# jmschrei/blueberry

Hardware: AMD Instinct MI355X
Metric: Gpair-updates/s per stress iteration, N=50k (higher is better)
Workload: dtype f32

## Files before the change

blueberry_amd/csrc/bb_solver.hip:

```cpp
#include <math.h>
#include <stddef.h>
#include <stdlib.h>
#include <string.h>
#include <time.h>
#include <unistd.h>

#include <algorithm>
#include <cmath>
#include <type_traits>
#include <vector>

#include <condition_variable>
#include <map>
#include <mutex>
#include <thread>
#include <tuple>

#include "bb_comm.h"
#include "bb_common.h"
#include "bb_group_barrier.h"
#include "bb_solver_kernels.h"

struct bb_solver {
    int dtype = BB_F32, device = 0, rank = 0, world = 1;
    bool wide = true;
    bb_layout_info L{};
    std::vector<int32_t> tile_I, tile_J;
    int64_t u_begin = 0, u_end = 0, n_local = 0;
    int64_t t_first = 0, n_local_tiles = 0;
    std::vector<int2> udesc;

    hipStream_t stream = nullptr;
    bool own_stream = false;
    bool stream_stuck = false;

    void *d_units = nullptr, *d_X = nullptr, *d_V = nullptr, *d_part = nullptr, *d_exch = nullptr;
    double momentum = 0.0;
    bool own_exch = false;
    int2 *d_udesc = nullptr;
    int chunk_q = 0, chunk_r = 0;
    bool nontemporal = true;
    char *d_arena = nullptr;
    int2 *d_wave_slots = nullptr;
    int lds_wave_floats = 0;
    double *d_stresspart = nullptr;
    double *d_stress_slot = nullptr;
    std::vector<int32_t> slot_strip;
    std::vector<int32_t> wave_last_strip;
    int n_maps = 1;
    void *d_bin_scale = nullptr;
    int *d_map_ptr = nullptr, *d_map_idx = nullptr;
    double *d_map_scalar = nullptr;
    std::vector<int64_t> map_begin;
    int64_t *d_red_lists = nullptr;
    int red_stride = 0, red_slices = 0;
    double *d_stress_hist = nullptr, *d_stress_scalar = nullptr;
    double *d_f64_tmp = nullptr;
    void *d_mv_in = nullptr;
    int64_t rowpart_elems = 0, colpart_elems = 0;
    int n_waves = 0, n_slots = 0;
    int wpb = 4;
    int dense_u0 = -1;
    int defer_cap_units = 0;
    int64_t defer_lds_bytes = 0;
    unsigned defer_attr_done = 0;
    int64_t hist_cap = 0, hist_n = 0;
    bool have_wish = false, have_coords = false, grad_pending = false;
    void *sum_target = nullptr;

    bb::Rccl::Comm comm = nullptr;
    bool comm_cached = false;
    bool comm_suspect = false;

    void *peer_arena = nullptr;
    int64_t peer_slot_elems = 0, peer_arena_bytes = 0;
    std::vector<void *> peer_mapped;
    std::vector<void *> peer_opened;
    void *d_peer_table = nullptr;
    void *d_peer_table_x = nullptr;
    bool peer_fused = true;
    PeerState *d_peer_state = nullptr;
    int peer_clock_khz = 100000;
    int peer_ranks_on_gpu = 1;
    unsigned *d_peer_mask = nullptr;
    unsigned *d_peer_counter = nullptr;
    unsigned long long peer_seq = 0;
    long long peer_limit_ticks = 0;
    bool peer_connected = false;

    bool row_owner = false;
    bool row_owner_built = false;
    bool bin_steps = false;
    int weight_power = 0;
    void *d_full = nullptr, *d_X2 = nullptr;
    int64_t full_ld = 0;
    double *d_ro_part = nullptr;
    int ro_blocks = 0, ro_wpr = 1;
    int64_t ro_launches = 0;

    bool timing = false;
    int timing_stride = 1;
    int64_t timing_iter = 0;
    std::vector<hipEvent_t> ev;
    size_t ev_used = 0;
};

namespace {

void comm_release(bb_solver *s, bool destroy);
int64_t peer_xpoison_offset(const bb_solver *s);

// ... 683 lines not shown
        }
    }
    if (rc == BB_OK) rc = bb_layout_rank_units(s->L.n_units, rank, world, &s->u_begin, &s->u_end);
    if (rc == BB_OK && tile_I == nullptr && s->u_end < ((int64_t)1 << 31)) {
        const char *e = getenv("BB_ARITH_DESC");
        if (!(e && atoi(e) == 0)) s->dense_u0 = (int)s->u_begin;
    }
    if (rc == BB_OK) {
        hipError_t e = bb::acquire_stream(device, &s->stream);
        if (e != hipSuccess)
            rc = bb::hip_status("hipStreamCreate", e);
        else
            s->own_stream = true;
    }
    if (rc == BB_OK) rc = build_indices(s);
    if (rc != BB_OK) {
        std::string keep = bb_last_error();
        bb_solver_destroy(s);
        bb::set_error(keep);
        return rc;
    }
    *out = s;
    return BB_OK;
}

int bb_solver_destroy(bb_solver *s) {
    if (!s) return BB_OK;
    hipSetDevice(s->device);
    if (!s->stream_stuck && (s->stream || !s->own_stream)) hipStreamSynchronize(s->stream);
    if (s->comm) {
        bb::Rccl::Comm c = s->comm;
        const bool cached = s->comm_cached, suspect = s->comm_suspect;
        comm_release(s, false);
        if (suspect) {
            if (bb::rccl().CommAbort) bb::rccl().CommAbort(c);
        } else if (!cached) {
            bb::rccl().CommDestroy(c);
        }
    }
    for (void *m : s->peer_opened) hipIpcCloseMemHandle(m);
    hipFree(s->peer_arena);
    hipFree(s->d_peer_table);
    hipFree(s->d_peer_table_x);
    hipFree(s->d_peer_state);
    hipFree(s->d_peer_counter);
    hipFree(s->d_peer_mask);
    for (hipEvent_t e : s->ev) hipEventDestroy(e);
    hipFree(s->d_arena);
    hipFree(s->d_bin_scale);
    hipFree(s->d_map_ptr);
    hipFree(s->d_map_idx);
    hipFree(s->d_map_scalar);
    if (s->own_exch) hipFree(s->d_exch);
    hipFree(s->d_mv_in);
    if (s->own_stream && s->stream && !s->stream_stuck) bb::release_stream(s->device, s->stream);
    delete s;
    (void)hipGetLastError();
    return BB_OK;
}

int bb_solver_set_stream(bb_solver *s, void *hip_stream) {
    BB_REQUIRE(s != nullptr, "bb_solver_set_stream: solver is NULL");
    BB_TRY(bb::enter_device(s->device));
    BB_HIP_CHECK(hipStreamSynchronize(s->stream));
    if (s->own_stream && s->stream) bb::release_stream(s->device, s->stream);
    s->stream = (hipStream_t)hip_stream;
    s->own_stream = false;
    return BB_OK;
}

int bb_solver_layout(const bb_solver *s, bb_layout_info *info, int64_t *u_begin, int64_t *u_end) {
    BB_REQUIRE(s != nullptr, "bb_solver_layout: solver is NULL");
    if (info) *info = s->L;
    if (u_begin) *u_begin = s->u_begin;
    if (u_end) *u_end = s->u_end;
    return BB_OK;
}

int bb_solver_set_wish_dense(bb_solver *s, const double *host, int64_t ld, int kind,
                             double alpha) {
    BB_REQUIRE(s != nullptr && host != nullptr, "bb_solver_set_wish_dense: NULL argument");
    BB_REQUIRE(ld >= s->L.n_bins, "bb_solver_set_wish_dense: ld < n_bins");
    BB_REQUIRE(kind == BB_KIND_WISH || kind == BB_KIND_COUNTS,
               "bb_solver_set_wish_dense: bad kind");
    BB_REQUIRE(kind == BB_KIND_WISH || alpha > 0.0, "bb_solver_set_wish_dense: alpha must be > 0");
    return set_wish_dense(s, host, ld, kind, alpha, 0, s->L.n_bins);
}

int bb_solver_set_maps(bb_solver *s, int n_maps, const int64_t *bin_begin, const double *lr_scale) {
    BB_REQUIRE(s != nullptr && bin_begin != nullptr && lr_scale != nullptr,
               "bb_solver_set_maps: NULL argument");
    BB_REQUIRE(n_maps >= 1 && n_maps <= s->L.n_blocks, "bb_solver_set_maps: bad n_maps");
    if (s->world != 1)
        return bb::fail(BB_ERR_STATE, "bb_solver_set_maps: one rank only (on several GPUs give every "
                                      "rank maps of its own)");
    const int64_t vw = s->L.vw, nb = s->L.n_blocks;
    BB_REQUIRE(bin_begin[0] == 0 && bin_begin[n_maps] == s->L.n_bins,
               "bb_solver_set_maps: bin_begin must run from 0 to n_bins");
    for (int m = 0; m < n_maps; ++m)
        BB_REQUIRE(bin_begin[m] % vw == 0 && bin_begin[m + 1] > bin_begin[m],
                   "bb_solver_set_maps: every map starts at a multiple of the tile edge and is not empty");
    BB_TRY(bb::enter_device(s->device));
    std::vector<int> map_of_block((size_t)nb, 0);
    for (int m = 0, b = 0; b < nb; ++b) {
        while (m + 1 < n_maps && (int64_t)b * vw >= bin_begin[m + 1]) ++m;
        map_of_block[(size_t)b] = m;
    }
// ... 880 lines not shown
int bb_solver_get_exchange_buffer(bb_solver *s, void **dev_ptr) {
    BB_REQUIRE(s != nullptr && dev_ptr != nullptr, "bb_solver_get_exchange_buffer: NULL argument");
    *dev_ptr = s->d_exch;
    return BB_OK;
}

int bb_solver_set_exchange_buffer(bb_solver *s, void *dev_ptr) {
    BB_REQUIRE(s != nullptr && dev_ptr != nullptr, "bb_solver_set_exchange_buffer: NULL argument");
    BB_TRY(bb::enter_device(s->device));
    BB_HIP_CHECK(hipStreamSynchronize(s->stream));
    if (s->own_exch) hipFree(s->d_exch);
    s->d_exch = dev_ptr;
    s->own_exch = false;
    return BB_OK;
}

int bb_solver_read_exchange(bb_solver *s, double *host, int64_t n) {
    BB_REQUIRE(s != nullptr && host != nullptr, "bb_solver_read_exchange: NULL argument");
    BB_REQUIRE(n == 3 * s->L.n_pad + 2, "bb_solver_read_exchange: n != exchange size");
    BB_TRY(bb::enter_device(s->device));
    double *tmp = nullptr;
    BB_TRY(dev_alloc(&tmp, n));
    hipError_t e = widen(s, s->d_exch, tmp, n);
    if (e == hipSuccess)
        e = hipMemcpyAsync(host, tmp, (size_t)n * sizeof(double), hipMemcpyDeviceToHost, s->stream);
    if (e == hipSuccess) e = hipStreamSynchronize(s->stream);
    hipFree(tmp);
    return bb::hip_status("bb_solver_read_exchange", e);
}

int bb_solver_write_exchange(bb_solver *s, const double *host, int64_t n) {
    BB_REQUIRE(s != nullptr && host != nullptr, "bb_solver_write_exchange: NULL argument");
    BB_REQUIRE(n == 3 * s->L.n_pad + 2, "bb_solver_write_exchange: n != exchange size");
    BB_TRY(bb::enter_device(s->device));
    double *tmp = nullptr;
    BB_TRY(dev_alloc(&tmp, n));
    hipError_t e = hipMemcpyAsync(tmp, host, (size_t)n * sizeof(double), hipMemcpyHostToDevice,
                                  s->stream);
    if (e == hipSuccess) e = narrow(s, tmp, s->d_exch, n);
    if (e == hipSuccess) e = hipStreamSynchronize(s->stream);
    hipFree(tmp);
    return bb::hip_status("bb_solver_write_exchange", e);
}

int bb_solver_matvec_sq(bb_solver *s, const double *x, double *y) {
    BB_REQUIRE(s != nullptr && x != nullptr && y != nullptr, "bb_solver_matvec_sq: NULL argument");
    if (!s->have_wish) return bb::fail(BB_ERR_STATE, "bb_solver_matvec_sq: no wish distances set");
    if (s->n_maps > 1)
        return bb::fail(BB_ERR_STATE, "bb_solver_matvec_sq: not for a solver of several maps");
    if (s->grad_pending)
        return bb::fail(BB_ERR_STATE, "bb_solver_matvec_sq: a bb_solver_grad is pending");
    BB_TRY(bb::enter_device(s->device));
    const int64_t n3 = s->L.n_pad * 3, es = bb::elem_size(s->dtype);
    if (!s->d_mv_in) BB_TRY(dev_alloc((char **)&s->d_mv_in, n3 * es));
    void *d_in = s->d_mv_in;
    hipError_t e = hipMemsetAsync(s->d_f64_tmp, 0, (size_t)n3 * 8, s->stream);
    if (e == hipSuccess)
        e = hipMemcpyAsync(s->d_f64_tmp, x, (size_t)s->L.n_bins * 24, hipMemcpyHostToDevice, s->stream);
    if (e == hipSuccess) e = narrow(s, s->d_f64_tmp, d_in, n3);
    int rc = BB_OK;
    if (e != hipSuccess) rc = bb::hip_status("bb_solver_matvec_sq", e);
    if (rc == BB_OK) rc = launch_grad(s, kOpMatvec2, d_in);
    if (rc == BB_OK) rc = launch_reduce(s, kReduceExchange, 0.0, nullptr, kScalePlainSum);
    if (rc == BB_OK) {
        e = widen(s, s->d_exch, s->d_f64_tmp, n3);
        if (e == hipSuccess)
            e = hipMemcpyAsync(y, s->d_f64_tmp, (size_t)s->L.n_bins * 24, hipMemcpyDeviceToHost,
                               s->stream);
        if (e == hipSuccess) e = hipStreamSynchronize(s->stream);
        if (e != hipSuccess)
            rc = bb::hip_status("bb_solver_matvec_sq", e);
    }
    if (hipStreamSynchronize(s->stream) != hipSuccess && rc == BB_OK)
        rc = bb::fail(BB_ERR_HIP, "bb_solver_matvec_sq: the stream did not drain");
    return rc;
}

int bb_solver_stress(bb_solver *s, double *stress) {
    BB_TRY(check_ready(s, "bb_solver_stress"));
    BB_REQUIRE(stress != nullptr, "bb_solver_stress: stress is NULL");
    BB_TRY(bb::enter_device(s->device));
    BB_TRY(launch_grad(s));
    if (s->n_maps > 1) {
        std::vector<double> per((size_t)s->n_maps);
        BB_TRY(launch_reduce(s, kReduceStressOnly, 0.0, s->d_map_scalar));
        BB_HIP_CHECK(hipStreamSynchronize(s->stream));
        BB_HIP_CHECK(hipMemcpy(per.data(), s->d_map_scalar, per.size() * sizeof(double),
                               hipMemcpyDeviceToHost));
        *stress = 0.0;
        for (double v : per) *stress += v;
        return BB_OK;
    }
    BB_TRY(launch_reduce(s, kReduceStressOnly, 0.0, s->d_stress_scalar));
    BB_HIP_CHECK(hipStreamSynchronize(s->stream));
    BB_HIP_CHECK(hipMemcpy(stress, s->d_stress_scalar, sizeof(double), hipMemcpyDeviceToHost));
    return BB_OK;
}

int bb_solver_stress_maps(bb_solver *s, double *stress, int n_maps) {
    BB_TRY(check_ready(s, "bb_solver_stress_maps"));
    BB_REQUIRE(stress != nullptr && n_maps == s->n_maps, "bb_solver_stress_maps: bad argument");
    BB_TRY(bb::enter_device(s->device));
    BB_TRY(launch_grad(s));
    double *out = s->n_maps > 1 ? s->d_map_scalar : s->d_stress_scalar;
    BB_TRY(launch_reduce(s, kReduceStressOnly, 0.0, out));
    BB_HIP_CHECK(hipStreamSynchronize(s->stream));
    BB_HIP_CHECK(hipMemcpy(stress, out, (size_t)s->n_maps * sizeof(double), hipMemcpyDeviceToHost));
// ... 147 lines not shown
    *ms_avg = ms / launches;
    return BB_OK;
}

int bb_solver_iteration_path(const bb_solver *s, int *row_owner, int *waves_per_row) {
    BB_REQUIRE(s != nullptr, "bb_solver_iteration_path: solver is NULL");
    if (row_owner) *row_owner = s->row_owner ? 1 : 0;
    if (waves_per_row) *waves_per_row = s->row_owner ? s->ro_wpr : 0;
    return BB_OK;
}

int bb_solver_traffic(const bb_solver *s, int64_t *unit_bytes, int64_t *pairs_dense) {
    BB_REQUIRE(s != nullptr, "bb_solver_traffic: solver is NULL");
    if (unit_bytes) *unit_bytes = s->n_local * bb::kUnitBytes;
    if (pairs_dense) *pairs_dense = s->L.n_bins * (s->L.n_bins - 1) / 2;
    return BB_OK;
}

}

namespace {

void jacobi3(double *a, double *z) {
    for (int q = 0; q < 9; ++q) z[q] = (q % 4 == 0) ? 1.0 : 0.0;
    for (int sweep = 0; sweep < 50; ++sweep) {
        const double off = a[1] * a[1] + a[2] * a[2] + a[5] * a[5];
        if (off < 1e-300) break;
        for (int p = 0; p < 3; ++p)
            for (int q = p + 1; q < 3; ++q) {
                const double apq = a[p * 3 + q];
                if (apq == 0.0) continue;
                const double theta = (a[q * 3 + q] - a[p * 3 + p]) / (2.0 * apq);
                const double t = (theta >= 0 ? 1.0 : -1.0) / (fabs(theta) + sqrt(theta * theta + 1.0));
                const double c = 1.0 / sqrt(t * t + 1.0), sn = t * c;
                for (int k = 0; k < 3; ++k) {
                    const double akp = a[k * 3 + p], akq = a[k * 3 + q];
                    a[k * 3 + p] = c * akp - sn * akq;
                    a[k * 3 + q] = sn * akp + c * akq;
                }
                for (int k = 0; k < 3; ++k) {
                    const double apk = a[p * 3 + k], aqk = a[q * 3 + k];
                    a[p * 3 + k] = c * apk - sn * aqk;
                    a[q * 3 + k] = sn * apk + c * aqk;
                }
                for (int k = 0; k < 3; ++k) {
                    const double zkp = z[k * 3 + p], zkq = z[k * 3 + q];
                    z[k * 3 + p] = c * zkp - sn * zkq;
                    z[k * 3 + q] = sn * zkp + c * zkq;
                }
            }
    }
}

template <typename T>
int spectral_init_t(TypeTag<T>, bb_solver *s, int n_iter, const double *v0, double tol, int *iters_done,
                    double *residual_out) {
    const int64_t n = s->L.n_bins, n_pad = s->L.n_pad, n3 = n_pad * 3;
    if (!s->d_mv_in) BB_TRY(dev_alloc((char **)&s->d_mv_in, n3 * (int64_t)sizeof(T)));
    bb::DevBuf bV, bZ, bS, bP, bF;
    if (bV.alloc((size_t)n3 * 8) != hipSuccess || bZ.alloc((size_t)n3 * 8) != hipSuccess ||
        bS.alloc(24 * 8) != hipSuccess || bP.alloc((size_t)2 * kSpMaxGroups * 12 * 8) != hipSuccess ||
        bF.alloc(sizeof(int)) != hipSuccess)
        return bb::fail(BB_ERR_NOMEM, "bb_solver_spectral_init: out of device memory");
    double *dV = (double *)bV.p, *dZ = (double *)bZ.p, *dS = (double *)bS.p;
    double *dP0 = (double *)bP.p, *dP1 = dP0 + kSpMaxGroups * 12;
    int *dF = (int *)bF.p;
    hipStream_t st = s->stream;
    const dim3 gvec((unsigned)((n_pad + kSpWG - 1) / kSpWG)), bwg(kSpWG);
    const int groups = (int)std::min<int64_t>(kSpMaxGroups, (n_pad + kSpWG - 1) / kSpWG);
    const dim3 ggrp((unsigned)groups);
    const Affine3 ident = {{0, 0, 0}, {1, 0, 0, 0, 1, 0, 0, 0, 1}, 1.0};
    double sums[12];
    auto fetch_sums = [&]() -> int {
        BB_HIP_CHECK(hipStreamSynchronize(st));
        BB_HIP_CHECK(hipMemcpy(sums, dS, sizeof(sums), hipMemcpyDeviceToHost));
        return BB_OK;
    };
    auto orthonormalise = [&]() -> int {
        BB_HIP_CHECK(bb::launch(sp_affine_stats_kernel<double>, ggrp, bwg, 0, st, (const double *)dZ, dV,
                                n, n_pad, (const double *)dP1, groups, (int)kSpChol, 1.0, dF, dP0));
        BB_HIP_CHECK(bb::launch(sp_affine_centre_kernel<T>, gvec, bwg, 0, st, (const double *)dV, dV,
                                (T *)s->d_mv_in, n, n_pad, (const double *)dP0, groups, dF));
        return BB_OK;
    };
    auto apply_B = [&]() -> int {
        BB_TRY(launch_grad(s, kOpMatvec2, s->d_mv_in));
        BB_TRY(exchange_sum(s));
        BB_HIP_CHECK(bb::launch(sp_stats_kernel<T>, ggrp, bwg, 0, st, (const T *)s->d_exch, n, n_pad, dP0));
        BB_HIP_CHECK(bb::launch(sp_affine_stats_kernel<T>, ggrp, bwg, 0, st, (const T *)s->d_exch, dZ, n,
                                n_pad, (const double *)dP0, groups, (int)kSpMean, -0.5, dF, dP1));
        return BB_OK;
    };
    BB_HIP_CHECK(hipMemsetAsync(dF, 0, sizeof(int), st));
    BB_HIP_CHECK(hipMemsetAsync(s->d_V, 0, (size_t)n3 * sizeof(T), st));
    BB_HIP_CHECK(hipMemsetAsync(dZ, 0, (size_t)n3 * 8, st));
    BB_HIP_CHECK(hipMemcpyAsync(dZ, v0, (size_t)n * 24, hipMemcpyHostToDevice, st));
    BB_HIP_CHECK(bb::launch(sp_stats_kernel<double>, ggrp, bwg, 0, st, (const double *)dZ, n, n_pad, dP1));
    BB_TRY(orthonormalise());
    double zsums[12];
    double residual = -1.0;
    int done = 0;
    bool have_product = false;
    for (int it = 0; it < n_iter; ++it) {
        BB_TRY(apply_B());
        if (tol > 0.0 && it > 0) {
            BB_HIP_CHECK(bb::launch(gram3_kernel<double, double>, dim3(1), dim3(1024), 0, st,
                                    (const double *)dV, (const double *)dZ, n, dS));
            BB_HIP_CHECK(bb::launch(sp_fold_partials_kernel, dim3(1), dim3(64), 0, st,
                                    (const double *)dP1, groups, dS + 12));
            BB_TRY(fetch_sums());
            BB_HIP_CHECK(hipMemcpy(zsums, dS + 12, sizeof(zsums), hipMemcpyDeviceToHost));
            double gg = 0.0;
            const double zz = zsums[0] + zsums[4] + zsums[8];
            for (int q = 0; q < 9; ++q) gg += sums[q] * sums[q];
            residual = zz > 0.0 ? sqrt(std::max(0.0, zz - gg) / zz) : 0.0;
            if (residual < tol) { have_product = true; break; }
        }
        BB_TRY(orthonormalise());
        done = it + 1;
    }
    if (iters_done) *iters_done = done;
    if (residual_out) *residual_out = residual;
    if (!have_product) {
        BB_TRY(apply_B());
        BB_HIP_CHECK(bb::launch(gram3_kernel<double, double>, dim3(1), dim3(1024), 0, st,
                                (const double *)dV, (const double *)dZ, n, dS));
        BB_TRY(fetch_sums());
    }
    int lost = 0;
    BB_HIP_CHECK(hipMemcpy(&lost, dF, sizeof(int), hipMemcpyDeviceToHost));
    if (lost)
        return bb::fail(BB_ERR_STATE, "bb_solver_spectral_init: the iterate lost rank "
                                      "(fewer than 3 independent directions in the map)");
    double m[9], z[9];
    for (int i = 0; i < 3; ++i)
        for (int j = 0; j < 3; ++j) m[i * 3 + j] = 0.5 * (sums[i * 3 + j] + sums[j * 3 + i]);
    jacobi3(m, z);
    int order[3] = {0, 1, 2};
    std::sort(order, order + 3, [&](int a, int b) { return m[a * 4] > m[b * 4]; });
    BB_HIP_CHECK(hipMemsetAsync(dZ, 0, (size_t)n3 * 8, st));
    BB_HIP_CHECK(hipMemcpyAsync(dZ, v0, (size_t)n * 24, hipMemcpyHostToDevice, st));
    BB_HIP_CHECK(bb::launch(gram3_kernel<double, double>, dim3(1), dim3(1024), 0, st, (const double *)dV,
                            (const double *)dZ, n, dS));
    BB_TRY(fetch_sums());
    Affine3 f = ident;
    for (int c = 0; c < 3; ++c) {
        const double lam = m[order[c] * 4] > 0.0 ? m[order[c] * 4] : 0.0;
        double side = 0.0;
        for (int r = 0; r < 3; ++r) side += z[r * 3 + order[c]] * sums[r * 3];
        const double sg = side < 0.0 ? -1.0 : 1.0;
        for (int r = 0; r < 3; ++r) f.m[r * 3 + c] = sg * z[r * 3 + order[c]] * sqrt(lam);
    }
    BB_HIP_CHECK(bb::launch(affine3_kernel<double, T>, dim3((unsigned)((n_pad + 255) / 256)), dim3(256), 0,
                            st, (const double *)dV, (T *)s->d_X, n, n_pad, f));
    BB_HIP_CHECK(hipMemsetAsync(s->d_V, 0, (size_t)n3 * sizeof(T), st));
    BB_HIP_CHECK(hipStreamSynchronize(st));
    return BB_OK;
}

}

extern "C" int bb_solver_spectral_init_tol(bb_solver *s, int n_iter, double tol, const double *v0,
                                           int *iters_done, double *residual);
extern "C" int bb_solver_spectral_init(bb_solver *s, int n_iter, const double *v0) {
    return bb_solver_spectral_init_tol(s, n_iter, 0.0, v0, nullptr, nullptr);
}
extern "C" int bb_solver_spectral_init_tol(bb_solver *s, int n_iter, double tol, const double *v0,
                                           int *iters_done, double *residual) {
    BB_REQUIRE(s != nullptr && v0 != nullptr, "bb_solver_spectral_init: NULL argument");
    BB_REQUIRE(n_iter >= 0 && n_iter <= 100000, "bb_solver_spectral_init: bad n_iter");
    BB_REQUIRE(tol >= 0.0 && tol < 1.0, "bb_solver_spectral_init: need 0 <= tol < 1");
    if (!s->have_wish) return bb::fail(BB_ERR_STATE, "bb_solver_spectral_init: no wish distances set");
    if (s->world != 1 && !s->peer_connected && !s->comm)
        return bb::fail(BB_ERR_STATE, "bb_solver_spectral_init: with world > 1 the ranks need their "
                                      "exchange first (bb_solver_peer_connect, or bb_solver_comm_init "
                                      "/ _attach); without one the caller sums bb_solver_matvec_sq "
                                      "over the ranks");
    if (s->grad_pending)
        return bb::fail(BB_ERR_STATE, "bb_solver_spectral_init: a bb_solver_grad is pending");
    if (s->n_maps > 1)
        return bb::fail(BB_ERR_STATE, "bb_solver_spectral_init: not for a solver of several maps "
                                      "(start each map with a solver of its own)");
    BB_REQUIRE(s->L.n_bins >= 3, "bb_solver_spectral_init: needs at least 3 bins");
    BB_TRY(bb::enter_device(s->device));
    BB_TRY(by_dtype(s, [&](auto t) { return spectral_init_t(t, s, n_iter, v0, tol, iters_done, residual); }));
    s->have_coords = true;
    s->hist_n = 0;
    s->grad_pending = false;
    return BB_OK;
}

namespace {

constexpr int kGroupAborted = -1;

}

struct bb_group {
    std::vector<bb_solver *> m;
    std::vector<void *> exch;
    std::vector<void *> d_src;
    std::vector<unsigned *> d_mask;
// ... 221 lines not shown
```

blueberry_amd/csrc/bb_solver_kernels.h:

```cpp
#pragma once

#include <hip/hip_runtime.h>
#include <stdint.h>

#include <type_traits>

#include "blueberry_hip.h"

namespace {


template <typename T>
struct Traits;
template <>
struct Traits<float> {
    using Vec = float4;
    static constexpr int VPL = 4;
    static __device__ __forceinline__ float eps2() { return 1e-30f; }
};
template <>
struct Traits<double> {
    using Vec = double2;
    static constexpr int VPL = 2;
    static __device__ __forceinline__ double eps2() { return 1e-300; }
// ... 1528 lines not shown
    const int b = (int)(i / VW);
    const int n_blocks = (int)((n_bins + VW - 1) / VW);
    const int i0 = (int)(i - i % RPU), r = (int)(i % RPU);
    double acc = 0.0;
    for (int J = b; J < n_blocks; ++J) {
        const int64_t ul = lower(J * VW, i0);
        if (ul >= n_local || udesc[ul].y != J * VW || udesc[ul].x != i0) continue;
        const T *row = units + ul * (RPU * VW) + (int64_t)r * VW;
        for (int c = lane; c < VW; c += 64) {
            const int64_t j = (int64_t)J * VW + c;
            if (j > i && j < n_bins) acc += weight(row[c]);
        }
    }
    const int c = (int)(i - (int64_t)b * VW);
    for (int64_t p = lane; p * RPU < i; p += 64) {
        const int64_t ul = lower(b * VW, (int)(p * RPU));
        if (ul >= n_local || udesc[ul].y != b * VW || udesc[ul].x != (int)(p * RPU)) continue;
        const T *col = units + ul * (RPU * VW) + c;
        for (int q = 0; q < RPU; ++q)
            if (p * RPU + q < i) acc += weight(col[q * VW]);
    }
    acc = wave_sum_hi(acc);
    if (lane == 63) sums[i] = acc;
}

template <bool NT>
__global__ __launch_bounds__(256, 4) void stream_read_kernel(const float4 *__restrict__ units,
                                                             int chunk_q, int chunk_r,
                                                             float *__restrict__ sink) {
    const int lane = threadIdx.x & 63;
    const int w = __builtin_amdgcn_readfirstlane(blockIdx.x * 4 + (threadIdx.x >> 6));
    const int ua = w * chunk_q + (w < chunk_r ? w : chunk_r);
    const int ub = ua + chunk_q + (w < chunk_r ? 1 : 0);
    float4 acc = make_float4(0.f, 0.f, 0.f, 0.f);
    if (ua < ub) {
        float4 d[8];
        const float4 *first = units + (int64_t)ua * 512 + lane;
#pragma unroll
        for (int r = 0; r < 8; ++r) d[r] = stream_load<NT>(first + r * 64);
        for (int u = ua; u < ub; ++u) {
            const int un = u + 1 < ub ? u + 1 : u;
            const float4 *next = units + (int64_t)un * 512 + lane;
#pragma unroll
            for (int r = 0; r < 8; ++r) {
                acc.x += d[r].x; acc.y += d[r].y; acc.z += d[r].z; acc.w += d[r].w;
                d[r] = stream_load<NT>(next + r * 64);
                __builtin_amdgcn_sched_barrier(0);
            }
        }
    }
    if (acc.x + acc.y + acc.z + acc.w == 12345.678f) sink[w] = acc.x;
}

template <typename TA, typename TB>
__global__ __launch_bounds__(1024) void gram3_kernel(const TA *__restrict__ A,
                                                     const TB *__restrict__ B, int64_t n,
                                                     double *__restrict__ out) {
    __shared__ double sh[12][16];
    double acc[12];
#pragma unroll
    for (int q = 0; q < 12; ++q) acc[q] = 0.0;
    for (int64_t i = threadIdx.x; i < n; i += 1024) {
        const double a0 = (double)A[3 * i], a1 = (double)A[3 * i + 1], a2 = (double)A[3 * i + 2];
        const double b0 = (double)B[3 * i], b1 = (double)B[3 * i + 1], b2 = (double)B[3 * i + 2];
        acc[0] = fma(a0, b0, acc[0]); acc[1] = fma(a0, b1, acc[1]); acc[2] = fma(a0, b2, acc[2]);
        acc[3] = fma(a1, b0, acc[3]); acc[4] = fma(a1, b1, acc[4]); acc[5] = fma(a1, b2, acc[5]);
        acc[6] = fma(a2, b0, acc[6]); acc[7] = fma(a2, b1, acc[7]); acc[8] = fma(a2, b2, acc[8]);
        acc[9] += a0; acc[10] += a1; acc[11] += a2;
    }
    const int lane = threadIdx.x & 63, wv = threadIdx.x >> 6;
#pragma unroll
    for (int q = 0; q < 12; ++q) {
        double v = acc[q];
#pragma unroll
        for (int off = 32; off > 0; off >>= 1) v += __shfl_down(v, off, 64);
        if (lane == 0) sh[q][wv] = v;
    }
    __syncthreads();
    if (threadIdx.x < 12) {
        double v = 0.0;
        for (int k = 0; k < 16; ++k) v += sh[threadIdx.x][k];
        out[threadIdx.x] = v;
    }
}

struct Affine3 {
    double mean[3], m[9], scale;
};
template <typename TI, typename TO>
__global__ __launch_bounds__(256) void affine3_kernel(const TI *__restrict__ in, TO *__restrict__ out,
                                                      int64_t n_bins, int64_t n_pad, Affine3 a) {
    const int64_t i = (int64_t)blockIdx.x * 256 + threadIdx.x;
    if (i >= n_pad) return;
    double o0 = 0.0, o1 = 0.0, o2 = 0.0;
    if (i < n_bins) {
        const double x0 = (double)in[3 * i] - a.mean[0], x1 = (double)in[3 * i + 1] - a.mean[1],
                     x2 = (double)in[3 * i + 2] - a.mean[2];
        o0 = a.scale * (x0 * a.m[0] + x1 * a.m[3] + x2 * a.m[6]);
        o1 = a.scale * (x0 * a.m[1] + x1 * a.m[4] + x2 * a.m[7]);
        o2 = a.scale * (x0 * a.m[2] + x1 * a.m[5] + x2 * a.m[8]);
    }
    out[3 * i] = (TO)o0; out[3 * i + 1] = (TO)o1; out[3 * i + 2] = (TO)o2;
}

constexpr int kSpWG = 256;
constexpr int kSpMaxGroups = 256;

__device__ __forceinline__ void sp_rows(int64_t n_pad, int64_t &r0, int64_t &r1) {
    const int64_t per = (n_pad + gridDim.x - 1) / gridDim.x;
    r0 = (int64_t)blockIdx.x * per;
    r1 = r0 + per < n_pad ? r0 + per : n_pad;
}
__device__ __forceinline__ void sp_store_partial(double (&acc)[12], double *__restrict__ partial) {
    __shared__ double sh[12][kSpWG / 64];
    const int lane = threadIdx.x & 63, wv = threadIdx.x >> 6;
#pragma unroll
    for (int q = 0; q < 12; ++q) {
        double v = acc[q];
#pragma unroll
        for (int off = 32; off > 0; off >>= 1) v += __shfl_down(v, off, 64);
        if (lane == 0) sh[q][wv] = v;
    }
    __syncthreads();
    if (threadIdx.x < 12) {
        double v = 0.0;
#pragma unroll
        for (int k = 0; k < kSpWG / 64; ++k) v += sh[threadIdx.x][k];
        partial[(int64_t)blockIdx.x * 12 + threadIdx.x] = v;
    }
}
__device__ __forceinline__ void sp_accumulate(double (&acc)[12], double a0, double a1, double a2) {
    acc[0] = fma(a0, a0, acc[0]); acc[1] = fma(a0, a1, acc[1]); acc[2] = fma(a0, a2, acc[2]);
    acc[3] = fma(a1, a0, acc[3]); acc[4] = fma(a1, a1, acc[4]); acc[5] = fma(a1, a2, acc[5]);
    acc[6] = fma(a2, a0, acc[6]); acc[7] = fma(a2, a1, acc[7]); acc[8] = fma(a2, a2, acc[8]);
    acc[9] += a0; acc[10] += a1; acc[11] += a2;
}

template <typename TI>
__global__ __launch_bounds__(kSpWG) void sp_stats_kernel(const TI *__restrict__ in, int64_t n_bins,
                                                         int64_t n_pad, double *__restrict__ partial) {
    int64_t r0, r1;
    sp_rows(n_pad, r0, r1);
    double acc[12];
#pragma unroll
    for (int q = 0; q < 12; ++q) acc[q] = 0.0;
    for (int64_t i = r0 + threadIdx.x; i < r1 && i < n_bins; i += kSpWG)
        sp_accumulate(acc, (double)in[3 * i], (double)in[3 * i + 1], (double)in[3 * i + 2]);
    sp_store_partial(acc, partial);
}

__global__ __launch_bounds__(64) void sp_fold_partials_kernel(const double *__restrict__ partial,
                                                              int groups, double *__restrict__ out) {
    if (threadIdx.x >= 12) return;
    double v = 0.0;
    for (int g = 0; g < groups; ++g) v += partial[(int64_t)g * 12 + threadIdx.x];
    out[threadIdx.x] = v;
}

__host__ __device__ inline bool sp_chol3_inv_upper(const double *g, double *rinv) {
    double r[9] = {0, 0, 0, 0, 0, 0, 0, 0, 0};
    for (int j = 0; j < 3; ++j) {
        double d = g[j * 3 + j];
        for (int k = 0; k < j; ++k) d -= r[k * 3 + j] * r[k * 3 + j];
        if (!(d > 0.0)) return false;
        r[j * 3 + j] = sqrt(d);
        for (int c = j + 1; c < 3; ++c) {
            double v = g[j * 3 + c];
            for (int k = 0; k < j; ++k) v -= r[k * 3 + j] * r[k * 3 + c];
            r[j * 3 + c] = v / r[j * 3 + j];
        }
    }
    for (int q = 0; q < 9; ++q) rinv[q] = 0.0;
    for (int j = 0; j < 3; ++j) {
        rinv[j * 3 + j] = 1.0 / r[j * 3 + j];
        for (int i = j - 1; i >= 0; --i) {
            double v = 0.0;
            for (int k = i + 1; k <= j; ++k) v -= r[i * 3 + k] * rinv[k * 3 + j];
            rinv[i * 3 + j] = v / r[i * 3 + i];
        }
    }
    return true;
}

enum { kSpMean = 0, kSpChol = 1, kSpCholMean = 2 };
__device__ __forceinline__ void sp_map_from_partials(const double *__restrict__ partial, int groups,
                                                     int64_t n_bins, int mode, double scale,
                                                     int *__restrict__ flag, Affine3 &A, Affine3 &B) {
    __shared__ double tot[12];
    __shared__ Affine3 maps[2];
    const int t = threadIdx.x;
    if (t < 192) {
        const int q = t >> 4, l = t & 15;
        double v = 0.0;
        for (int g = l; g < groups; g += 16) v += partial[(int64_t)g * 12 + q];
#pragma unroll
        for (int off = 8; off > 0; off >>= 1) v += __shfl_xor(v, off, 16);
        if (l == 0) tot[q] = v;
    }
    __syncthreads();
    if (t == 0) {
        Affine3 a, b;
        for (int k = 0; k < 3; ++k) a.mean[k] = 0.0;
        for (int k = 0; k < 9; ++k) a.m[k] = (k % 4 == 0) ? 1.0 : 0.0;
        a.scale = 1.0;
        b = a;
        if (mode == kSpMean) {
            for (int k = 0; k < 3; ++k) a.mean[k] = tot[9 + k] / (double)n_bins;
            a.scale = scale;
        } else {
            double rinv[9];
            if (!sp_chol3_inv_upper(tot, rinv)) {
                *flag = 1;
            } else {
                for (int k = 0; k < 9; ++k) a.m[k] = rinv[k];
                b = a;
                const double m0 = tot[9] / (double)n_bins, m1 = tot[10] / (double)n_bins,
                             m2 = tot[11] / (double)n_bins;
                b.mean[0] = m0 * rinv[0] + m1 * rinv[3] + m2 * rinv[6];
                b.mean[1] = m0 * rinv[1] + m1 * rinv[4] + m2 * rinv[7];
                b.mean[2] = m0 * rinv[2] + m1 * rinv[5] + m2 * rinv[8];
            }
        }
        maps[0] = a;
        maps[1] = b;
    }
    __syncthreads();
    A = maps[0];
    B = maps[1];
}

template <typename TI>
__global__ __launch_bounds__(kSpWG) void sp_affine_stats_kernel(const TI *in, double *out,
                                                                int64_t n_bins, int64_t n_pad,
                                                                const double *__restrict__ partial_in,
                                                                int groups, int mode, double scale,
                                                                int *__restrict__ flag,
                                                                double *__restrict__ partial) {
    Affine3 A, unused;
    sp_map_from_partials(partial_in, groups, n_bins, mode, scale, flag, A, unused);
    int64_t r0, r1;
    sp_rows(n_pad, r0, r1);
    double acc[12];
#pragma unroll
    for (int q = 0; q < 12; ++q) acc[q] = 0.0;
    for (int64_t i = r0 + threadIdx.x; i < r1; i += kSpWG) {
        double o0 = 0.0, o1 = 0.0, o2 = 0.0;
        if (i < n_bins) {
            const double x0 = (double)in[3 * i] - A.mean[0], x1 = (double)in[3 * i + 1] - A.mean[1],
                         x2 = (double)in[3 * i + 2] - A.mean[2];
            o0 = A.scale * (x0 * A.m[0] + x1 * A.m[3] + x2 * A.m[6]);
            o1 = A.scale * (x0 * A.m[1] + x1 * A.m[4] + x2 * A.m[7]);
            o2 = A.scale * (x0 * A.m[2] + x1 * A.m[5] + x2 * A.m[8]);
            sp_accumulate(acc, o0, o1, o2);
        }
        out[3 * i] = o0; out[3 * i + 1] = o1; out[3 * i + 2] = o2;
    }
    sp_store_partial(acc, partial);
}

template <typename T>
__global__ __launch_bounds__(kSpWG) void sp_affine_centre_kernel(const double *in, double *out_v,
                                                                 T *__restrict__ out_mv,
                                                                 int64_t n_bins, int64_t n_pad,
                                                                 const double *__restrict__ partial_in,
                                                                 int groups, int *__restrict__ flag) {
    Affine3 A, B;
    sp_map_from_partials(partial_in, groups, n_bins, kSpCholMean, 1.0, flag, A, B);
    const int64_t i = (int64_t)blockIdx.x * kSpWG + threadIdx.x;
    if (i >= n_pad) return;
    double o0 = 0.0, o1 = 0.0, o2 = 0.0, c0 = 0.0, c1 = 0.0, c2 = 0.0;
    if (i < n_bins) {
        const double x0 = in[3 * i], x1 = in[3 * i + 1], x2 = in[3 * i + 2];
        o0 = x0 * A.m[0] + x1 * A.m[3] + x2 * A.m[6];
        o1 = x0 * A.m[1] + x1 * A.m[4] + x2 * A.m[7];
        o2 = x0 * A.m[2] + x1 * A.m[5] + x2 * A.m[8];
        c0 = o0 - B.mean[0]; c1 = o1 - B.mean[1]; c2 = o2 - B.mean[2];
    }
    out_v[3 * i] = o0; out_v[3 * i + 1] = o1; out_v[3 * i + 2] = o2;
    out_mv[3 * i] = (T)c0; out_mv[3 * i + 1] = (T)c1; out_mv[3 * i + 2] = (T)c2;
}

template <typename T>
__global__ void f64_to_T_kernel(const double *__restrict__ in, T *__restrict__ out, int64_t n) {
    const int64_t e = (int64_t)blockIdx.x * 256 + threadIdx.x;
    if (e < n) out[e] = (T)in[e];
}
template <typename T>
__global__ void T_to_f64_kernel(const T *__restrict__ in, double *__restrict__ out, int64_t n) {
    const int64_t e = (int64_t)blockIdx.x * 256 + threadIdx.x;
    if (e < n) out[e] = (double)in[e];
}

}
```

Measured before the change: 1643.

## Fuse spectral-init Gram reductions into affine stats kernel and cache scratch buffers

```diff
diff --git a/blueberry_amd/csrc/bb_solver.hip b/blueberry_amd/csrc/bb_solver.hip
--- a/blueberry_amd/csrc/bb_solver.hip
+++ b/blueberry_amd/csrc/bb_solver.hip
@@ -57,6 +57,9 @@
     double *d_stress_hist = nullptr, *d_stress_scalar = nullptr;
     double *d_f64_tmp = nullptr;
     void *d_mv_in = nullptr;
+    bool mv_in_own = false;
+    char *d_sp = nullptr;
+    double *h_sp = nullptr;
     int64_t rowpart_elems = 0, colpart_elems = 0;
     int n_waves = 0, n_slots = 0;
     int wpb = 4;
@@ -846,7 +849,9 @@
     hipFree(s->d_map_idx);
     hipFree(s->d_map_scalar);
     if (s->own_exch) hipFree(s->d_exch);
-    hipFree(s->d_mv_in);
+    if (s->mv_in_own) hipFree(s->d_mv_in);
+    hipFree(s->d_sp);
+    hipHostFree(s->h_sp);
     if (s->own_stream && s->stream && !s->stream_stuck) bb::release_stream(s->device, s->stream);
     delete s;
     (void)hipGetLastError();
@@ -1833,7 +1838,10 @@
         return bb::fail(BB_ERR_STATE, "bb_solver_matvec_sq: a bb_solver_grad is pending");
     BB_TRY(bb::enter_device(s->device));
     const int64_t n3 = s->L.n_pad * 3, es = bb::elem_size(s->dtype);
-    if (!s->d_mv_in) BB_TRY(dev_alloc((char **)&s->d_mv_in, n3 * es));
+    if (!s->d_mv_in) {
+        BB_TRY(dev_alloc((char **)&s->d_mv_in, n3 * es));
+        s->mv_in_own = true;
+    }
     void *d_in = s->d_mv_in;
     hipError_t e = hipMemsetAsync(s->d_f64_tmp, 0, (size_t)n3 * 8, s->stream);
     if (e == hipSuccess)
@@ -2087,64 +2095,111 @@
     }
 }
 
+struct SpScratch {
+    double *V, *Z, *p, *P0, *P1, *Pg;
+    int *flag;
+    void *mv_in;
+    int64_t read_words, bytes;
+};
+SpScratch sp_layout(char *base, int64_t n_pad, int groups, int64_t elem_size) {
+    SpScratch sc;
+    int64_t off = 0;
+    auto take = [&](int64_t bytes) {
+        void *at = (void *)((uintptr_t)base + (uintptr_t)off);
+        off += (bytes + 255) / 256 * 256;
+        return at;
+    };
+    sc.V = (double *)take(n_pad * 24);
+    sc.Z = (double *)take(n_pad * 24);
+    sc.p = (double *)take(n_pad * 8);
+    sc.P0 = (double *)take((int64_t)groups * 12 * 8);
+    sc.read_words = 2 * (int64_t)groups * 12 + 1;
+    sc.P1 = (double *)take(sc.read_words * 8);
+    sc.Pg = sc.P1 + (int64_t)groups * 12;
+    sc.flag = (int *)(sc.Pg + (int64_t)groups * 12);
+    sc.mv_in = take(n_pad * 3 * elem_size);
+    sc.bytes = off;
+    return sc;
+}
+
 template <typename T>
 int spectral_init_t(TypeTag<T>, bb_solver *s, int n_iter, const double *v0, double tol, int *iters_done,
                     double *residual_out) {
     const int64_t n = s->L.n_bins, n_pad = s->L.n_pad, n3 = n_pad * 3;
-    if (!s->d_mv_in) BB_TRY(dev_alloc((char **)&s->d_mv_in, n3 * (int64_t)sizeof(T)));
-    bb::DevBuf bV, bZ, bS, bP, bF;
-    if (bV.alloc((size_t)n3 * 8) != hipSuccess || bZ.alloc((size_t)n3 * 8) != hipSuccess ||
-        bS.alloc(24 * 8) != hipSuccess || bP.alloc((size_t)2 * kSpMaxGroups * 12 * 8) != hipSuccess ||
-        bF.alloc(sizeof(int)) != hipSuccess)
-        return bb::fail(BB_ERR_NOMEM, "bb_solver_spectral_init: out of device memory");
-    double *dV = (double *)bV.p, *dZ = (double *)bZ.p, *dS = (double *)bS.p;
-    double *dP0 = (double *)bP.p, *dP1 = dP0 + kSpMaxGroups * 12;
-    int *dF = (int *)bF.p;
     hipStream_t st = s->stream;
     const dim3 gvec((unsigned)((n_pad + kSpWG - 1) / kSpWG)), bwg(kSpWG);
     const int groups = (int)std::min<int64_t>(kSpMaxGroups, (n_pad + kSpWG - 1) / kSpWG);
     const dim3 ggrp((unsigned)groups);
+    if (!s->d_sp) {
+        const SpScratch want = sp_layout(nullptr, n_pad, groups, (int64_t)sizeof(T));
+        char *block = nullptr;
+        double *words = nullptr;
+        BB_TRY(dev_alloc(&block, want.bytes));
+        if (hipHostMalloc((void **)&words, (size_t)want.read_words * 8, hipHostMallocDefault) != hipSuccess) {
+            hipFree(block);
+            return bb::fail(BB_ERR_NOMEM, "bb_solver_spectral_init: out of pinned host memory");
+        }
+        if (s->mv_in_own) hipFree(s->d_mv_in);
+        s->d_sp = block;
+        s->h_sp = words;
+        s->d_mv_in = sp_layout(block, n_pad, groups, (int64_t)sizeof(T)).mv_in;
+        s->mv_in_own = false;
+    }
+    const SpScratch sc = sp_layout(s->d_sp, n_pad, groups, (int64_t)sizeof(T));
+    double *dV = sc.V, *dZ = sc.Z, *dP0 = sc.P0, *dP1 = sc.P1;
+    int *dF = sc.flag;
     const Affine3 ident = {{0, 0, 0}, {1, 0, 0, 0, 1, 0, 0, 0, 1}, 1.0};
-    double sums[12];
-    auto fetch_sums = [&]() -> int {
-        BB_HIP_CHECK(hipStreamSynchronize(st));
-        BB_HIP_CHECK(hipMemcpy(sums, dS, sizeof(sums), hipMemcpyDeviceToHost));
-        return BB_OK;
-    };
     auto orthonormalise = [&]() -> int {
-        BB_HIP_CHECK(bb::launch(sp_affine_stats_kernel<double>, ggrp, bwg, 0, st, (const double *)dZ, dV,
-                                n, n_pad, (const double *)dP1, groups, (int)kSpChol, 1.0, dF, dP0));
+        BB_HIP_CHECK(bb::launch(sp_affine_stats_kernel<double, false>, ggrp, bwg, 0, st, (const double *)dZ,
+                                dV, n, n_pad, (const double *)dP1, groups, (int)kSpChol, 1.0, dF, dP0,
+                                nullptr, nullptr, nullptr));
         BB_HIP_CHECK(bb::launch(sp_affine_centre_kernel<T>, gvec, bwg, 0, st, (const double *)dV, dV,
                                 (T *)s->d_mv_in, n, n_pad, (const double *)dP0, groups, dF));
         return BB_OK;
     };
-    auto apply_B = [&]() -> int {
+    auto apply_B = [&](bool may_be_last) -> int {
         BB_TRY(launch_grad(s, kOpMatvec2, s->d_mv_in));
         BB_TRY(exchange_sum(s));
-        BB_HIP_CHECK(bb::launch(sp_stats_kernel<T>, ggrp, bwg, 0, st, (const T *)s->d_exch, n, n_pad, dP0));
-        BB_HIP_CHECK(bb::launch(sp_affine_stats_kernel<T>, ggrp, bwg, 0, st, (const T *)s->d_exch, dZ, n,
-                                n_pad, (const double *)dP0, groups, (int)kSpMean, -0.5, dF, dP1));
+        BB_HIP_CHECK(bb::launch(sp_stats_kernel<T, false>, ggrp, bwg, 0, st, (const T *)s->d_exch, n, n_pad,
+                                dP0, nullptr));
+        BB_HIP_CHECK(bb::launch(sp_affine_stats_kernel<T, true>, ggrp, bwg, 0, st, (const T *)s->d_exch, dZ,
+                                n, n_pad, (const double *)dP0, groups, (int)kSpMean, -0.5, dF, dP1,
+                                (const double *)dV, may_be_last ? (const double *)sc.p : nullptr, sc.Pg));
         return BB_OK;
     };
-    BB_HIP_CHECK(hipMemsetAsync(dF, 0, sizeof(int), st));
+    double sums[12], zsums[12];
+    int lost = 0;
+    auto read_sums = [&]() -> int {
+        BB_HIP_CHECK(hipMemcpyAsync(s->h_sp, dP1, (size_t)sc.read_words * 8, hipMemcpyDeviceToHost, st));
+        BB_HIP_CHECK(hipStreamSynchronize(st));
+        const double *hz = s->h_sp, *hg = hz + (int64_t)groups * 12;
+        for (int q = 0; q < 12; ++q) {
+            double z = 0.0, g = 0.0;
+            for (int k = 0; k < groups; ++k) {
+                z += hz[k * 12 + q];
+                g += hg[k * 12 + q];
+            }
+            zsums[q] = z;
+            sums[q] = g;
+        }
+        memcpy(&lost, hg + (int64_t)groups * 12, sizeof(int));
+        return BB_OK;
+    };
+    BB_HIP_CHECK(hipMemsetAsync(dF, 0, 8, st));
     BB_HIP_CHECK(hipMemsetAsync(s->d_V, 0, (size_t)n3 * sizeof(T), st));
-    BB_HIP_CHECK(hipMemsetAsync(dZ, 0, (size_t)n3 * 8, st));
+    if (n_pad > n) BB_HIP_CHECK(hipMemsetAsync(dZ + 3 * n, 0, (size_t)(n_pad - n) * 24, st));
     BB_HIP_CHECK(hipMemcpyAsync(dZ, v0, (size_t)n * 24, hipMemcpyHostToDevice, st));
-    BB_HIP_CHECK(bb::launch(sp_stats_kernel<double>, ggrp, bwg, 0, st, (const double *)dZ, n, n_pad, dP1));
+    BB_HIP_CHECK(bb::launch(sp_stats_kernel<double, true>, ggrp, bwg, 0, st, (const double *)dZ, n, n_pad,
+                            dP1, sc.p));
     BB_TRY(orthonormalise());
-    double zsums[12];
     double residual = -1.0;
     int done = 0;
     bool have_product = false;
     for (int it = 0; it < n_iter; ++it) {
-        BB_TRY(apply_B());
-        if (tol > 0.0 && it > 0) {
-            BB_HIP_CHECK(bb::launch(gram3_kernel<double, double>, dim3(1), dim3(1024), 0, st,
-                                    (const double *)dV, (const double *)dZ, n, dS));
-            BB_HIP_CHECK(bb::launch(sp_fold_partials_kernel, dim3(1), dim3(64), 0, st,
-                                    (const double *)dP1, groups, dS + 12));
-            BB_TRY(fetch_sums());
-            BB_HIP_CHECK(hipMemcpy(zsums, dS + 12, sizeof(zsums), hipMemcpyDeviceToHost));
+        const bool check = tol > 0.0 && it > 0;
+        BB_TRY(apply_B(check));
+        if (check) {
+            BB_TRY(read_sums());
             double gg = 0.0;
             const double zz = zsums[0] + zsums[4] + zsums[8];
             for (int q = 0; q < 9; ++q) gg += sums[q] * sums[q];
@@ -2157,13 +2212,9 @@
     if (iters_done) *iters_done = done;
     if (residual_out) *residual_out = residual;
     if (!have_product) {
-        BB_TRY(apply_B());
-        BB_HIP_CHECK(bb::launch(gram3_kernel<double, double>, dim3(1), dim3(1024), 0, st,
-                                (const double *)dV, (const double *)dZ, n, dS));
-        BB_TRY(fetch_sums());
-    }
-    int lost = 0;
-    BB_HIP_CHECK(hipMemcpy(&lost, dF, sizeof(int), hipMemcpyDeviceToHost));
+        BB_TRY(apply_B(true));
+        BB_TRY(read_sums());
+    }
     if (lost)
         return bb::fail(BB_ERR_STATE, "bb_solver_spectral_init: the iterate lost rank "
                                       "(fewer than 3 independent directions in the map)");
@@ -2173,16 +2224,11 @@
     jacobi3(m, z);
     int order[3] = {0, 1, 2};
     std::sort(order, order + 3, [&](int a, int b) { return m[a * 4] > m[b * 4]; });
-    BB_HIP_CHECK(hipMemsetAsync(dZ, 0, (size_t)n3 * 8, st));
-    BB_HIP_CHECK(hipMemcpyAsync(dZ, v0, (size_t)n * 24, hipMemcpyHostToDevice, st));
-    BB_HIP_CHECK(bb::launch(gram3_kernel<double, double>, dim3(1), dim3(1024), 0, st, (const double *)dV,
-                            (const double *)dZ, n, dS));
-    BB_TRY(fetch_sums());
     Affine3 f = ident;
     for (int c = 0; c < 3; ++c) {
         const double lam = m[order[c] * 4] > 0.0 ? m[order[c] * 4] : 0.0;
         double side = 0.0;
-        for (int r = 0; r < 3; ++r) side += z[r * 3 + order[c]] * sums[r * 3];
+        for (int r = 0; r < 3; ++r) side += z[r * 3 + order[c]] * sums[9 + r];
         const double sg = side < 0.0 ? -1.0 : 1.0;
         for (int r = 0; r < 3; ++r) f.m[r * 3 + c] = sg * z[r * 3 + order[c]] * sqrt(lam);
     }
diff --git a/blueberry_amd/csrc/bb_solver_kernels.h b/blueberry_amd/csrc/bb_solver_kernels.h
--- a/blueberry_amd/csrc/bb_solver_kernels.h
+++ b/blueberry_amd/csrc/bb_solver_kernels.h
@@ -1604,38 +1604,6 @@
     if (acc.x + acc.y + acc.z + acc.w == 12345.678f) sink[w] = acc.x;
 }
 
-template <typename TA, typename TB>
-__global__ __launch_bounds__(1024) void gram3_kernel(const TA *__restrict__ A,
-                                                     const TB *__restrict__ B, int64_t n,
-                                                     double *__restrict__ out) {
-    __shared__ double sh[12][16];
-    double acc[12];
-#pragma unroll
-    for (int q = 0; q < 12; ++q) acc[q] = 0.0;
-    for (int64_t i = threadIdx.x; i < n; i += 1024) {
-        const double a0 = (double)A[3 * i], a1 = (double)A[3 * i + 1], a2 = (double)A[3 * i + 2];
-        const double b0 = (double)B[3 * i], b1 = (double)B[3 * i + 1], b2 = (double)B[3 * i + 2];
-        acc[0] = fma(a0, b0, acc[0]); acc[1] = fma(a0, b1, acc[1]); acc[2] = fma(a0, b2, acc[2]);
-        acc[3] = fma(a1, b0, acc[3]); acc[4] = fma(a1, b1, acc[4]); acc[5] = fma(a1, b2, acc[5]);
-        acc[6] = fma(a2, b0, acc[6]); acc[7] = fma(a2, b1, acc[7]); acc[8] = fma(a2, b2, acc[8]);
-        acc[9] += a0; acc[10] += a1; acc[11] += a2;
-    }
-    const int lane = threadIdx.x & 63, wv = threadIdx.x >> 6;
-#pragma unroll
-    for (int q = 0; q < 12; ++q) {
-        double v = acc[q];
-#pragma unroll
-        for (int off = 32; off > 0; off >>= 1) v += __shfl_down(v, off, 64);
-        if (lane == 0) sh[q][wv] = v;
-    }
-    __syncthreads();
-    if (threadIdx.x < 12) {
-        double v = 0.0;
-        for (int k = 0; k < 16; ++k) v += sh[threadIdx.x][k];
-        out[threadIdx.x] = v;
-    }
-}
-
 struct Affine3 {
     double mean[3], m[9], scale;
 };
@@ -1688,25 +1656,21 @@
     acc[9] += a0; acc[10] += a1; acc[11] += a2;
 }
 
-template <typename TI>
+template <typename TI, bool KEEP_P>
 __global__ __launch_bounds__(kSpWG) void sp_stats_kernel(const TI *__restrict__ in, int64_t n_bins,
-                                                         int64_t n_pad, double *__restrict__ partial) {
+                                                         int64_t n_pad, double *__restrict__ partial,
+                                                         double *__restrict__ p) {
     int64_t r0, r1;
     sp_rows(n_pad, r0, r1);
     double acc[12];
 #pragma unroll
     for (int q = 0; q < 12; ++q) acc[q] = 0.0;
-    for (int64_t i = r0 + threadIdx.x; i < r1 && i < n_bins; i += kSpWG)
-        sp_accumulate(acc, (double)in[3 * i], (double)in[3 * i + 1], (double)in[3 * i + 2]);
+    for (int64_t i = r0 + threadIdx.x; i < r1 && i < n_bins; i += kSpWG) {
+        const double a0 = (double)in[3 * i];
+        if (KEEP_P) p[i] = a0;
+        sp_accumulate(acc, a0, (double)in[3 * i + 1], (double)in[3 * i + 2]);
+    }
     sp_store_partial(acc, partial);
-}
-
-__global__ __launch_bounds__(64) void sp_fold_partials_kernel(const double *__restrict__ partial,
-                                                              int groups, double *__restrict__ out) {
-    if (threadIdx.x >= 12) return;
-    double v = 0.0;
-    for (int g = 0; g < groups; ++g) v += partial[(int64_t)g * 12 + threadIdx.x];
-    out[threadIdx.x] = v;
 }
 
 __host__ __device__ inline bool sp_chol3_inv_upper(const double *g, double *rinv) {
@@ -1781,20 +1745,23 @@
     B = maps[1];
 }
 
-template <typename TI>
+template <typename TI, bool GRAM>
 __global__ __launch_bounds__(kSpWG) void sp_affine_stats_kernel(const TI *in, double *out,
                                                                 int64_t n_bins, int64_t n_pad,
                                                                 const double *__restrict__ partial_in,
                                                                 int groups, int mode, double scale,
                                                                 int *__restrict__ flag,
-                                                                double *__restrict__ partial) {
+                                                                double *__restrict__ partial,
+                                                                const double *__restrict__ V,
+                                                                const double *__restrict__ p,
+                                                                double *__restrict__ partial_g) {
     Affine3 A, unused;
     sp_map_from_partials(partial_in, groups, n_bins, mode, scale, flag, A, unused);
     int64_t r0, r1;
     sp_rows(n_pad, r0, r1);
-    double acc[12];
-#pragma unroll
-    for (int q = 0; q < 12; ++q) acc[q] = 0.0;
+    double acc[12], gacc[12];
+#pragma unroll
+    for (int q = 0; q < 12; ++q) acc[q] = gacc[q] = 0.0;
     for (int64_t i = r0 + threadIdx.x; i < r1; i += kSpWG) {
         double o0 = 0.0, o1 = 0.0, o2 = 0.0;
         if (i < n_bins) {
@@ -1804,10 +1771,25 @@
             o1 = A.scale * (x0 * A.m[1] + x1 * A.m[4] + x2 * A.m[7]);
             o2 = A.scale * (x0 * A.m[2] + x1 * A.m[5] + x2 * A.m[8]);
             sp_accumulate(acc, o0, o1, o2);
+            if (GRAM) {
+                const double v0 = V[3 * i], v1 = V[3 * i + 1], v2 = V[3 * i + 2];
+                gacc[0] = fma(v0, o0, gacc[0]); gacc[1] = fma(v0, o1, gacc[1]); gacc[2] = fma(v0, o2, gacc[2]);
+                gacc[3] = fma(v1, o0, gacc[3]); gacc[4] = fma(v1, o1, gacc[4]); gacc[5] = fma(v1, o2, gacc[5]);
+                gacc[6] = fma(v2, o0, gacc[6]); gacc[7] = fma(v2, o1, gacc[7]); gacc[8] = fma(v2, o2, gacc[8]);
+                if (p) {
+                    const double pi = p[i];
+                    gacc[9] = fma(v0, pi, gacc[9]); gacc[10] = fma(v1, pi, gacc[10]);
+                    gacc[11] = fma(v2, pi, gacc[11]);
+                }
+            }
         }
         out[3 * i] = o0; out[3 * i + 1] = o1; out[3 * i + 2] = o2;
     }
     sp_store_partial(acc, partial);
+    if (GRAM) {
+        __syncthreads();
+        sp_store_partial(gacc, partial_g);
+    }
 }
 
 template <typename T>
```

New measurement: 1644 (median of 2 runs). About the same (+0.1%).
